# wxwilcke/mrgcn

Measured on AMD Instinct MI355X. Metric: full-batch R-GCN epoch time (ms), AM-shaped graph, lower is better.
Workload: dtype f32

## Files before the change

### mrgcn_amd/csrc/rgcn_fused.hip

```cpp
#include <cmath>
#include <cstdlib>

#include <mutex>
#include <unordered_map>

#include "common.hpp"
#include "config.hpp"

namespace mrgcn {
namespace {

constexpr int kTB = 256;
constexpr int kMixTB = 512;
constexpr int kMixFwdTB = 1024;
constexpr int kPre = 8;

__host__ __device__ constexpr int comp_stride(int BT) { return BT >= 4 ? BT + 4 : BT; }

template <int BT>
__device__ __forceinline__ void load_comp_row(const float *row, float (&w)[BT]) {
  if constexpr (BT % 4 == 0) {
#pragma unroll
    for (int b = 0; b < BT; b += 4) {
      const float4 q = *reinterpret_cast<const float4 *>(row + b);
      w[b] = q.x; w[b + 1] = q.y; w[b + 2] = q.z; w[b + 3] = q.w;
    }
  } else {
#pragma unroll
    for (int b = 0; b < BT; ++b) w[b] = row[b];
  }
}

template <int BT, typename OT>
__global__ __launch_bounds__(kMixFwdTB) void k_mix_fwd(const int32_t *__restrict__ nptr,
                                                    const int32_t *__restrict__ urel,
                                                    const int32_t *__restrict__ mpos,
                                                    const float *__restrict__ V,
                                                    const float *__restrict__ comp, int64_t N, int R,
                                                    int B, int b0, int F,
                                                    const float *__restrict__ addend, int64_t ldA,
                                                    OT *__restrict__ M, int64_t ldM, int accumulate,
                                                    int comp_in_lds,
                                                    const int32_t *__restrict__ node_ids = nullptr) {
  extern __shared__ __align__(16) float s_comp[];
  constexpr int CS = comp_stride(BT);
  const int nb = min(BT, B - b0);
  if (comp_in_lds) {
    for (int t = threadIdx.x; t < R * BT; t += blockDim.x) {
      int r = t / BT, b = t - r * BT;
      s_comp[r * CS + b] = (b < nb) ? comp[(int64_t)r * B + b0 + b] : 0.f;
    }
    __syncthreads();
  }
  const int64_t total = N * F;
  for (int64_t t = (int64_t)blockIdx.x * blockDim.x + threadIdx.x; t < total;
       t += (int64_t)gridDim.x * blockDim.x) {
    const int64_t j = t / F;
    const int o = (int)(t - j * F);
    const int32_t c0 = nptr[j], c1 = nptr[j + 1];
    if (c0 == c1) continue;
    float v[BT];
    const int64_t jv = node_ids ? (int64_t)node_ids[j] : j;
#pragma unroll
    for (int b = 0; b < BT; ++b)
      v[b] = (o < F && b < nb) ? V[(jv * B + (b0 + b)) * F + o] : 0.f;

    for (int32_t cb = c0; cb < c1; cb += kPre) {
      int rr[kPre];
      int32_t pp[kPre];
      float aa[kPre];
#pragma unroll
      for (int i = 0; i < kPre; ++i) {
        const int32_t c = (cb + i < c1) ? cb + i : cb;
        rr[i] = urel[c];
        pp[i] = mpos ? mpos[c] : c;
        aa[i] = addend ? addend[(int64_t)c * ldA + o] : 0.f;
      }
#pragma unroll
      for (int i = 0; i < kPre; ++i) {
        if (cb + i < c1) {
          float s = aa[i];
          if (comp_in_lds) {
            float w[BT];
            load_comp_row<BT>(s_comp + rr[i] * CS, w);
#pragma unroll
            for (int b = 0; b < BT; ++b) s = fmaf(w[b], v[b], s);
          } else {
            const float *cr = comp + (int64_t)rr[i] * B + b0;
#pragma unroll
            for (int b = 0; b < BT; ++b)
              if (b < nb) s = fmaf(cr[b], v[b], s);
          }
          OT *m = M + (int64_t)pp[i] * ldM + o;
          if (accumulate) s += load_operand<OT>(m);
          if constexpr (sizeof(OT) == 2) {
            const float next = __shfl_down(s, 1, kWave);
            if ((o & 1) == 0 && (F & 1) == 0) {
              *reinterpret_cast<uint32_t *>(m) = (uint32_t)f32_to_bf16(s) | ((uint32_t)f32_to_bf16(next) << 16);
            } else if (F & 1) {
              store_operand<OT>(m, s);
            }
          } else {
            store_operand<OT>(m, s);
          }
        }
      }
    }
  }
}

__device__ __forceinline__ void wave_lds_fence() {
  __builtin_amdgcn_fence(__ATOMIC_ACQ_REL, "wavefront");
  __builtin_amdgcn_wave_barrier();
}

using f32x4m = __attribute__((ext_vector_type(4))) float;
constexpr int kFwdTB = 1024;

template <int KS, bool NEAR, int ADD, typename OT, typename AT = float>
__device__ __forceinline__ void mix_node_tiles(int32_t c0, int32_t c1, int32_t base, int32_t ur, int32_t mp,
                                               const float (&pa)[4], const int32_t *__restrict__ urel,
                                               const int32_t *__restrict__ mpos, const float *s_comp,
                                               const float *s_v, int B, int F, const AT *__restrict__ addend,
                                               int64_t ldA, OT *__restrict__ M, int64_t ldM, int m, int kq,
                                               const AT *s_add = nullptr) {
  constexpr int KP = KS * 16 + 4;
  f32x4m bv[KS];
#pragma unroll
  for (int ks = 0; ks < KS; ++ks) {
    const int k0 = ks * 16 + 4 * kq;
    const float *t = s_v + k0 * F + m;
    bv[ks].x = (m < F && k0 + 0 < B) ? t[0] : 0.f;
    bv[ks].y = (m < F && k0 + 1 < B) ? t[F] : 0.f;
    bv[ks].z = (m < F && k0 + 2 < B) ? t[2 * F] : 0.f;
    bv[ks].w = (m < F && k0 + 3 < B) ? t[3 * F] : 0.f;
  }
  for (int32_t cb = c0; cb < c1; cb += 16) {
    const int32_t cm = cb + m;
    int32_t r;
    int32_t pos[4];
    f32x4m acc = f32x4m{0.f, 0.f, 0.f, 0.f};
    if (NEAR) {
      r = __shfl(ur, (cm - base) & 63);
#pragma unroll
      for (int reg = 0; reg < 4; ++reg) {
        pos[reg] = __shfl(mp, (cb - base + 4 * kq + reg) & 63);
        if (ADD == 1) acc[reg] = pa[reg];
        if (ADD == 2) acc[reg] = load_operand<AT>(s_add + (min(cb + 4 * kq + reg, c1 - 1) - base) * (int)ldA + min(m, F - 1));
      }
    } else {
      r = urel[min(cm, c1 - 1)];
#pragma unroll
      for (int reg = 0; reg < 4; ++reg) {
        const int32_t c = min(cb + 4 * kq + reg, c1 - 1);
        pos[reg] = mpos ? mpos[c] : c;
        if (ADD) acc[reg] = load_operand<AT>(addend + (int64_t)c * ldA + min(m, F - 1));
      }
    }
#pragma unroll
    for (int ks = 0; ks < KS; ++ks) {
      f32x4m av = *reinterpret_cast<const f32x4m *>(s_comp + r * KP + ks * 16 + 4 * kq);
      if (cm >= c1) av = f32x4m{0.f, 0.f, 0.f, 0.f};
      acc = __builtin_amdgcn_mfma_f32_16x16x4f32(av.x, bv[ks].x, acc, 0, 0, 0);
      acc = __builtin_amdgcn_mfma_f32_16x16x4f32(av.y, bv[ks].y, acc, 0, 0, 0);
      acc = __builtin_amdgcn_mfma_f32_16x16x4f32(av.z, bv[ks].z, acc, 0, 0, 0);
      acc = __builtin_amdgcn_mfma_f32_16x16x4f32(av.w, bv[ks].w, acc, 0, 0, 0);
    }
    if (m < F) {
#pragma unroll
      for (int reg = 0; reg < 4; ++reg)
        if (cb + 4 * kq + reg < c1) store_operand<OT>(M + (int64_t)pos[reg] * ldM + m, acc[reg]);
    }
    if (NEAR && ADD == 1) break;
  }
}

template <int BT>
__global__ __launch_bounds__(256) void k_mix_fwd_wide(const int32_t *__restrict__ nptr, const int32_t *__restrict__ urel,
                                                      const int32_t *__restrict__ mpos, const float *__restrict__ V,
                                                      const float *__restrict__ comp, int64_t N, int R, int B, int F,
                                                      float *__restrict__ M, int64_t ldM,
                                                      const int32_t *__restrict__ node_ids) {
  extern __shared__ __align__(16) float s_comp[];
  for (int t = threadIdx.x; t < R * B; t += blockDim.x) s_comp[t] = comp[t];
  __syncthreads();
  const int lane = threadIdx.x & 63;
  const int wv = __builtin_amdgcn_readfirstlane((int)(threadIdx.x >> 6));
  const int f0 = 4 * lane;
  const bool active = f0 < F;
  const f32x4m zero = {0.f, 0.f, 0.f, 0.f};
  for (int64_t j = (int64_t)blockIdx.x * 4 + wv; j < N; j += (int64_t)gridDim.x * 4) {
    const int32_t c0 = nptr[j], c1 = nptr[j + 1];
    if (c0 == c1) continue;
    const int64_t jv = node_ids ? (int64_t)node_ids[j] : j;
    f32x4m v[BT];
#pragma unroll
    for (int b = 0; b < BT; ++b)
      v[b] = (active && b < B) ? *reinterpret_cast<const f32x4m *>(V + (jv * B + b) * F + f0) : zero;
    for (int32_t cb = c0; cb < c1; cb += 64) {
      const int32_t my = (cb + lane < c1) ? cb + lane : c1 - 1;
      const int32_t mr = urel[my], mp = mpos ? mpos[my] : my;
      const int cnt = (c1 - cb < 64) ? c1 - cb : 64;
      for (int t = 0; t < cnt; ++t) {
        const int r = __builtin_amdgcn_readlane(mr, t);
        const int64_t pos = __builtin_amdgcn_readlane(mp, t);
        f32x4m sum = zero;
#pragma unroll
        for (int b = 0; b < BT; ++b)
          if (b < B) sum += v[b] * s_comp[r * B + b];
        if (active) *reinterpret_cast<f32x4m *>(M + pos * ldM + f0) = sum;
      }
    }
  }
}

#ifndef MIX_V_NT
#define MIX_V_NT 1
#endif
constexpr int kAddPieces = 128;
constexpr int kMixTile = 4;
template <int KS, int NQ, int TN, int ADD, typename OT, bool IDS = false, typename AT = float, bool TK = false>
__global__ __launch_bounds__(kFwdTB) void k_mix_fwd_mfma(
    const int32_t *__restrict__ nptr, const int32_t *__restrict__ urel, const int32_t *__restrict__ mpos,
    const float *__restrict__ V, const float *__restrict__ comp, int64_t N, int R, int B, int F,
    const AT *__restrict__ addend, int64_t ldA, OT *__restrict__ M, int64_t ldM,
    const int32_t *__restrict__ node_ids = nullptr, unsigned long long *__restrict__ tickets = nullptr,
    int n_counters = 0, int tile = kMixTile) {
  extern __shared__ __align__(16) float s_mem[];
  constexpr int KP = KS * 16 + 4;
  float *s_comp = s_mem;
  const int BF = B * F, nf4 = BF >> 2;
  const int lane = threadIdx.x & 63;
  const int wv = __builtin_amdgcn_readfirstlane((int)(threadIdx.x >> 6));
  const int nw = blockDim.x >> 6;
  float *s_tile = s_mem + ((R * KP + 3) & ~3) + wv * (TN * BF);
  float *s_add = s_mem + ((R * KP + 3) & ~3) + nw * (TN * BF) + wv * (kAddPieces * 4);
  const int q4 = (int)((ldA * (int64_t)sizeof(AT)) >> 4);
  for (int t = threadIdx.x; t < R * KP; t += blockDim.x) {
    const int r = t / KP, k = t - r * KP;
    s_comp[t] = k < B ? comp[(int64_t)r * B + k] : 0.f;
  }
  __syncthreads();
  const int m = lane & 15, kq = lane >> 4;
  const int64_t ngroups = (N + TN - 1) / TN;
  const int64_t nwaves = (int64_t)gridDim.x * nw;
  int64_t g = (int64_t)blockIdx.x * nw + wv, g1 = g + nwaves, g2 = g + 2 * nwaves;
  unsigned long long *ctr = nullptr;
  int64_t seg_lo = 0, seg_hi = 0;
  unsigned long long tk_ahead = 0;
  auto tile_first = [&](unsigned long long t) {
    const int64_t st = seg_lo + (int64_t)t * tile;
    return st < seg_hi ? st : ngroups;
  };
  auto next_step = [&](int64_t x) {
    if (x >= ngroups) return x;
    if ((x - seg_lo + 1) % tile != 0 && x + 1 < seg_hi) return x + 1;
    const unsigned long long t = __shfl(tk_ahead, 0, 64);
    if (lane == 0) tk_ahead = atomicAdd(ctr, 1ull);
    return tile_first(t);
  };
  if (TK) {
    const int64_t wid = g;
    const int c = (int)(wid % n_counters);
    ctr = tickets + (int64_t)c * kWorkTicketStride;
    const int64_t per = ((ngroups + n_counters - 1) / n_counters + tile - 1) / tile * tile;
    seg_lo = (int64_t)c * per;
    seg_hi = min(seg_lo + per, ngroups);
    unsigned long long t0 = 0;
    if (lane == 0) {
      t0 = atomicAdd(ctr, 1ull);
      tk_ahead = atomicAdd(ctr, 1ull);
    }
    g = tile_first(__shfl(t0, 0, 64));
    g1 = next_step(g);
    g2 = next_step(g1);
  }
  if (g >= ngroups) return;
#define MIX_LOAD_NP(gg) nptr[min(min((gg), ngroups - 1) * TN + min(lane, TN), N)]
#define MIX_LOAD_ID(gg) (IDS ? node_ids[min(min((gg), ngroups - 1) * TN + min(lane, TN - 1), N - 1)] : 0)
#define MIX_LOAD_V(gg, idreg)                                                                               \
  _Pragma("unroll") for (int i = 0; i < TN; ++i) {                                                          \
    const int64_t nid = IDS ? (int64_t)__builtin_amdgcn_readlane(idreg, i) : min((gg) * TN + i, N - 1);     \
    const f32x4m *src = reinterpret_cast<const f32x4m *>(V) + nid * (int64_t)nf4;                           \
    _Pragma("unroll") for (int q = 0; q < NQ; ++q)                                                          \
      pv[i][q] = MIX_V_NT ? __builtin_nontemporal_load(src + min(lane + 64 * q, nf4 - 1)) : src[min(lane + 64 * q, nf4 - 1)]; \
  }
#define MIX_LOAD_IDX(np, ur, mp)                                                                            \
  {                                                                                                         \
    const int32_t a0 = __builtin_amdgcn_readlane(np, 0), a1 = __builtin_amdgcn_readlane(np, TN);            \
    const int32_t ci = max(min(a0 + lane, a1 - 1), 0);                                                      \
    ur = urel[ci];                                                                                          \
    mp = mpos ? mpos[ci] : ci;                                                                              \
    if (ADD == 2) {                                                                                         \
      const int64_t p0 = (int64_t)a0 * q4, p1 = (int64_t)a1 * q4;                                           \
      const f32x4m *a4 = reinterpret_cast<const f32x4m *>(addend);                                          \
      pa4_n1[0] = a4[max(min(p0 + lane, p1 - 1), (int64_t)0)];                                              \
      pa4_n1[1] = a4[max(min(p0 + 64 + lane, p1 - 1), (int64_t)0)];                                         \
    }                                                                                                       \
    if (ADD == 1) {                                                                                         \
      _Pragma("unroll") for (int i = 0; i < TN; ++i) {                                                      \
        const int32_t b0 = __builtin_amdgcn_readlane(np, i), b1 = __builtin_amdgcn_readlane(np, i + 1);     \
        _Pragma("unroll") for (int reg = 0; reg < 4; ++reg) pa_n1[i][reg] =                                 \
            load_operand<AT>(addend + (int64_t)max(min(b0 + 4 * kq + reg, b1 - 1), 0) * ldA + min(m, F - 1)); \
      }                                                                                                     \
    }                                                                                                       \
  }
  f32x4m pv[TN][NQ];
  f32x4m pa4_n1[2];
  float pa_n1[TN][4], pa_cur[TN][4];
  int32_t np_cur = MIX_LOAD_NP(g), np_n1 = MIX_LOAD_NP(g1);
  int32_t id_cur = MIX_LOAD_ID(g), id_n1 = MIX_LOAD_ID(g1);
  int32_t ur_cur, mp_cur, ur_n1, mp_n1;
  MIX_LOAD_IDX(np_cur, ur_n1, mp_n1)
  MIX_LOAD_V(g, id_cur)
  for (; g < ngroups; g = g1, g1 = g2, g2 = TK ? next_step(g2) : g2 + nwaves) {
    const int32_t np_now = np_cur;
    const int32_t cbase = __builtin_amdgcn_readlane(np_now, 0), cend = __builtin_amdgcn_readlane(np_now, TN);
    const int32_t np_n2 = MIX_LOAD_NP(g2);
    const int32_t id_n2 = MIX_LOAD_ID(g2);
    ur_cur = ur_n1;
    mp_cur = mp_n1;
    bool near = cend - cbase <= 64;
    if (ADD == 2) near = near && (cend - cbase) * q4 <= kAddPieces;
#pragma unroll
    for (int i = 0; i < TN; ++i) {
      if (ADD == 1) {
#pragma unroll
        for (int reg = 0; reg < 4; ++reg) pa_cur[i][reg] = pa_n1[i][reg];
        near = near && __builtin_amdgcn_readlane(np_now, i + 1) - __builtin_amdgcn_readlane(np_now, i) <= 16;
      }
      f32x4m *dst = reinterpret_cast<f32x4m *>(s_tile + i * BF);
#pragma unroll
      for (int q = 0; q < NQ; ++q)
        if (lane + 64 * q < nf4) dst[lane + 64 * q] = pv[i][q];
    }
    if (ADD == 2) {
      reinterpret_cast<f32x4m *>(s_add)[lane] = pa4_n1[0];
      reinterpret_cast<f32x4m *>(s_add)[64 + lane] = pa4_n1[1];
    }
    wave_lds_fence();
    MIX_LOAD_V(g1, id_n1)
    MIX_LOAD_IDX(np_n1, ur_n1, mp_n1)
    np_cur = np_n1;
    np_n1 = np_n2;
    id_n1 = id_n2;
    if (near) {
#pragma unroll
      for (int i = 0; i < TN; ++i) {
        const int32_t c0 = __builtin_amdgcn_readlane(np_now, i), c1 = __builtin_amdgcn_readlane(np_now, i + 1);
        if (c1 > c0)
          mix_node_tiles<KS, true, ADD, OT, AT>(c0, c1, cbase, ur_cur, mp_cur, pa_cur[i], urel, mpos, s_comp,
                                                s_tile + i * BF, B, F, addend, ldA, M, ldM, m, kq,
                                                reinterpret_cast<const AT *>(s_add));
      }
    } else {
#pragma unroll 1
      for (int i = 0; i < TN; ++i)
        mix_node_tiles<KS, false, ADD, OT, AT>(__builtin_amdgcn_readlane(np_now, i),
                                               __builtin_amdgcn_readlane(np_now, i + 1), cbase, ur_cur, mp_cur,
                                               pa_cur[0], urel, mpos, s_comp, s_tile + i * BF, B, F, addend, ldA, M,
                                               ldM, m, kq);
    }
    wave_lds_fence();
  }
#undef MIX_LOAD_NP
#undef MIX_LOAD_ID
#undef MIX_LOAD_V
#undef MIX_LOAD_IDX
}

template <int BT>
__global__ __launch_bounds__(kMixTB) void k_mix_bwd_dv(const int32_t *__restrict__ nptr,
                                                       const int32_t *__restrict__ urel,
                                                       const float *__restrict__ dM, int64_t ldM,
                                                       const float *__restrict__ comp, int64_t N, int R,
                                                       int B, int b0, int F, float *__restrict__ dV,
                                                       int comp_in_lds, double *__restrict__ sumsq) {
  extern __shared__ __align__(16) float s_comp[];
  float sq = 0.f;
  constexpr int CS = comp_stride(BT);
  const int nb = min(BT, B - b0);
  if (comp_in_lds) {
    for (int t = threadIdx.x; t < R * BT; t += blockDim.x) {
      int r = t / BT, b = t - r * BT;
      s_comp[r * CS + b] = (b < nb) ? comp[(int64_t)r * B + b0 + b] : 0.f;
    }
    __syncthreads();
  }
  const int64_t total = N * F;
  for (int64_t t = (int64_t)blockIdx.x * blockDim.x + threadIdx.x; t < total;
       t += (int64_t)gridDim.x * blockDim.x) {
    const int64_t j = t / F;
    const int o = (int)(t - j * F);
    const int32_t c0 = nptr[j], c1 = nptr[j + 1];
    float acc[BT];
#pragma unroll
    for (int b = 0; b < BT; ++b) acc[b] = 0.f;
    for (int32_t cb = c0; cb < c1; cb += kPre) {
      int rr[kPre];
      float dd[kPre];
#pragma unroll
      for (int i = 0; i < kPre; ++i) {
        const bool in = cb + i < c1;
        rr[i] = in ? urel[cb + i] : 0;
        dd[i] = in ? dM[(int64_t)(cb + i) * ldM + o] : 0.f;
      }
#pragma unroll
      for (int i = 0; i < kPre; ++i) {
        if (cb + i < c1) {
          if (comp_in_lds) {
            float w[BT];
            load_comp_row<BT>(s_comp + rr[i] * CS, w);
#pragma unroll
            for (int b = 0; b < BT; ++b) acc[b] = fmaf(w[b], dd[i], acc[b]);
          } else {
            const float *cr = comp + (int64_t)rr[i] * B + b0;
#pragma unroll
            for (int b = 0; b < BT; ++b)
              if (b < nb) acc[b] = fmaf(cr[b], dd[i], acc[b]);
          }
        }
      }
    }
#pragma unroll
    for (int b = 0; b < BT; ++b)
      if (b < nb) {
        dV[((int64_t)j * B + (b0 + b)) * F + o] = acc[b];
        sq = fmaf(acc[b], acc[b], sq);
      }
  }
  if (sumsq) {
    __shared__ float s_sq[kMixTB / 64];
#pragma unroll
    for (int off = 32; off > 0; off >>= 1) sq += __shfl_xor(sq, off, 64);
    if ((threadIdx.x & 63) == 0) s_sq[threadIdx.x >> 6] = sq;
    __syncthreads();
    if (threadIdx.x == 0) {
      float t = 0.f;
      for (int i = 0; i < (int)(blockDim.x >> 6); ++i) t += s_sq[i];
      atomicAdd(sumsq, (double)t);
    }
  }
}

constexpr int kNodeTB = 1024;
constexpr int kNodeLaunchTB = 512;
static_assert(kNodeLaunchTB % 64 == 0 && kNodeLaunchTB <= kNodeTB && 4 * kNodeLaunchTB <= 2048, "whole waves; four blocks per CU");
constexpr int kGroup = 4;

typedef float f32x4_a8 __attribute__((ext_vector_type(4), aligned(8)));
template <int FT>
__device__ __forceinline__ void load_row(const float *__restrict__ p, int F, float (&v)[FT]) {
  if ((F & 1) == 0) {
#pragma unroll
    for (int o = 0; o < FT; o += 4) {
      if (o + 4 <= F && o + 4 <= FT) {
        const f32x4_a8 t = *reinterpret_cast<const f32x4_a8 *>(p + o);
        v[o] = t.x;
        v[o + 1] = t.y;
        v[o + 2] = t.z;
        v[o + 3] = t.w;
      } else {
#pragma unroll
        for (int u = o; u < o + 4 && u < FT; u += 2) {
          if (u < F) {
            const float2 t = *reinterpret_cast<const float2 *>(p + u);
            v[u] = t.x;
            if (u + 1 < FT) v[u + 1] = t.y;
          } else {
            v[u] = 0.f;
            if (u + 1 < FT) v[u + 1] = 0.f;
          }
        }
      }
    }
  } else {
#pragma unroll
    for (int o = 0; o < FT; ++o) v[o] = (o < F) ? p[o] : 0.f;
  }
}
template <int FT>
__device__ __forceinline__ void store_row_f(float *__restrict__ p, int F, const float (&v)[FT]) {
  if ((F & 1) == 0) {
#pragma unroll
    for (int o = 0; o < FT; o += 2)
      if (o < F) *reinterpret_cast<float2 *>(p + o) = make_float2(v[o], (o + 1 < FT) ? v[o + 1] : 0.f);
  } else {
#pragma unroll
    for (int o = 0; o < FT; ++o)
      if (o < F) p[o] = v[o];
  }
}

template <int FT>
__global__ __launch_bounds__(kNodeTB) void k_mix_bwd_nm(const int32_t *__restrict__ nptr,
                                                        const int32_t *__restrict__ urel,
                                                        const float *__restrict__ dM, int64_t ldM,
                                                        const float *__restrict__ V,
                                                        const float *__restrict__ comp, int64_t N, int R,
                                                        int B, int F, float *__restrict__ dV,
                                                        float *__restrict__ dcomp,
                                                        double *__restrict__ sumsq, int top_rel,
                                                        const uint8_t *__restrict__ col_live,
                                                        uint8_t *__restrict__ node_cur, int dc_in_lds) {
  extern __shared__ __align__(16) float s_dc[];
  const int lane = threadIdx.x & 63;
  const int wv = __builtin_amdgcn_readfirstlane((int)(threadIdx.x >> 6));
  const int nw = blockDim.x >> 6;
  if (dc_in_lds) {
    for (int t = threadIdx.x; t < R * B; t += blockDim.x) s_dc[t] = 0.f;
    __syncthreads();
  }
  const bool on = lane < B;
  const int b = on ? lane : 0;
// ... 686 lines not shown
                                                      const int32_t *__restrict__ unode,
                                                      const float *__restrict__ X, int64_t ldX, int K,
                                                      const float *__restrict__ dM, int64_t ldM, int F,
                                                      float *__restrict__ dW) {
  extern __shared__ float smem[];
  const int chunk = blockIdx.x;
  const int r = relchunk_rel[chunk];
  const int32_t beg = relchunk_beg[chunk], end = relchunk_end[chunk];
  __shared__ int32_t s_c[kTK], s_j[kTK];
  const int XS = kKS + 1;
  float *Xs = smem;
  float *Ds = smem + kTK * XS;
  float *dWr = dW + (int64_t)r * K * F;

  for (int k0 = 0; k0 < K; k0 += kKS) {
    const int ks = min(kKS, K - k0);
    const int npairs = ks * F;
    for (int pbase = 0; pbase < npairs; pbase += kTB * kPP) {
      float acc[kPP];
#pragma unroll
      for (int q = 0; q < kPP; ++q) acc[q] = 0.f;
      for (int32_t t0 = beg; t0 < end; t0 += kTK) {
        const int nk = min(kTK, end - t0);
        __syncthreads();
        if (threadIdx.x < nk) {
          int32_t c = rperm[t0 + threadIdx.x];
          s_c[threadIdx.x] = c;
          s_j[threadIdx.x] = unode[c];
        }
        __syncthreads();
        for (int t = threadIdx.x; t < nk * ks; t += kTB) {
          int kk = t / ks, i = t - kk * ks;
          Xs[kk * XS + i] = X[(int64_t)s_j[kk] * ldX + k0 + i];
        }
        for (int t = threadIdx.x; t < nk * F; t += kTB) {
          int kk = t / F, o = t - kk * F;
          Ds[t] = dM[(int64_t)s_c[kk] * ldM + o];
        }
        __syncthreads();
#pragma unroll
        for (int q = 0; q < kPP; ++q) {
          const int p = pbase + q * kTB + threadIdx.x;
          if (p < npairs) {
            const int i = p / F, o = p - i * F;
            float s = acc[q];
            for (int kk = 0; kk < nk; ++kk) s = fmaf(Xs[kk * XS + i], Ds[kk * F + o], s);
            acc[q] = s;
          }
        }
      }
#pragma unroll
      for (int q = 0; q < kPP; ++q) {
        const int p = pbase + q * kTB + threadIdx.x;
        if (p < npairs) atomicAdd(&dWr[(int64_t)k0 * F + p], acc[q]);
      }
    }
  }
}

__global__ __launch_bounds__(kTB) void k_xform_bwd_dx(const int32_t *__restrict__ nptr,
                                                      const int32_t *__restrict__ urel,
                                                      const float *__restrict__ dM, int64_t ldM,
                                                      const float *__restrict__ W, int64_t N, int K,
                                                      int F, float *__restrict__ dX, int64_t lddX) {
  const int64_t total = N * K;
  for (int64_t t = (int64_t)blockIdx.x * blockDim.x + threadIdx.x; t < total;
       t += (int64_t)gridDim.x * blockDim.x) {
    const int64_t j = t / K;
    const int i = (int)(t - j * K);
    const int32_t c0 = nptr[j], c1 = nptr[j + 1];
    float s = 0.f;
    for (int32_t c = c0; c < c1; ++c) {
      const float *w = W + ((int64_t)urel[c] * K + i) * F;
      const float *dm = dM + (int64_t)c * ldM;
      for (int o = 0; o < F; ++o) s = fmaf(dm[o], w[o], s);
    }
    dX[j * lddX + i] = s;
  }
}

int grid_for(int64_t work_items, int tb = kTB, int max_blocks = 256 * 8) {
  int64_t b = (work_items + tb - 1) / tb;
  if (b < 1) b = 1;
  if (b > max_blocks) b = max_blocks;
  return (int)b;
}

constexpr size_t kLdsBudget = 64 * 1024;

bool use_mfma() {
  const bool v = cfg(CFG_XFORM_MFMA) != 0;
  return v;
}

int mix_grid(size_t lds, int64_t work_items) {
  int per_cu = lds > 0 ? (int)((160 * 1024) / (lds + 256)) : 4;
  if (per_cu > 4) per_cu = 4;
  if (per_cu < 1) per_cu = 1;
  int64_t want = (work_items + kMixTB - 1) / kMixTB;
  int64_t grid = 256 * per_cu * 2;
  if (grid > want) grid = want;
  return (int)(grid < 1 ? 1 : grid);
}

}
}

using namespace mrgcn;

namespace {

struct MixCols {
  const int32_t *nptr, *urel, *mpos, *node_ids;
  int64_t N, ncols;
  int R;
  unsigned long long *tickets = nullptr;
};

template <typename OT, typename AT = float>
int mix_fwd_cols(const MixCols *p, const float *V, const float *comp, int32_t B, int32_t F,
                 const AT *addend, int64_t ldA, OT *M, int64_t ldM, void *stream) {
  MRGCN_REQUIRE(V && comp && M, "NULL");
  MRGCN_REQUIRE(B > 0 && F > 0 && ldM >= F, "B / F / ldM");
  MRGCN_REQUIRE(!addend || ldA >= F, "ldA");
  if (p->ncols == 0 || p->N == 0) return MRGCN_OK;
  hipStream_t s = (hipStream_t)stream;
  const int R = p->R;
  const int64_t N = p->N;
  const int32_t *node_ids = p->node_ids;
  const int32_t *mpos_arg = p->mpos;
  if constexpr (sizeof(OT) == 4) {
    const bool wide_on = cfg(CFG_MIX_WIDE) != 0;
    if (wide_on && !addend && F > 16 && F <= 256 && F % 4 == 0 && B <= 4 && ldM % 4 == 0 &&
        ((((uintptr_t)V) | ((uintptr_t)M)) & 15) == 0 && (size_t)R * B * sizeof(float) <= 64 * 1024) {
      const size_t lds = (size_t)R * B * sizeof(float);
      int64_t grid = (N + 3) / 4;
      if (grid > 256 * 8) grid = 256 * 8;
#define MIXW_GO(BT_)                                                                                            \
  k_mix_fwd_wide<BT_><<<dim3((unsigned)grid), dim3(256), lds, s>>>(p->nptr, p->urel, mpos_arg, V, comp, N, R, B, F, \
                                                                    (float *)M, ldM, node_ids)
      if (B == 1) MIXW_GO(1);
      else if (B == 2) MIXW_GO(2);
      else MIXW_GO(4);
#undef MIXW_GO
      MRGCN_HIP_TRY(hipGetLastError());
      return MRGCN_OK;
    }
  }
  {
    const bool mfma_on = cfg(CFG_MIX_MFMA) != 0;
    constexpr int tn = 2;
    const int KS = (B + 15) / 16;
    const int NQ = (B * F + 255) / 256;
    const size_t lds_plain =
        ((size_t)((R * (KS * 16 + 4) + 3) & ~3) + (size_t)(kFwdTB / 64) * tn * B * F) * sizeof(float);
    const size_t lds_add = (size_t)(kFwdTB / 64) * kAddPieces * 4 * sizeof(float);
    const bool add_vec = addend && (ldA * sizeof(AT)) % 16 == 0 && ldA <= 16 && (((uintptr_t)addend) & 15) == 0 &&
                         !node_ids && cfg(CFG_MIX_ADD_VEC) != 0 &&
                         lds_plain + lds_add <= 150 * 1024;
    const size_t lds = lds_plain + (add_vec ? lds_add : 0);
    if (mfma_on && B <= 64 && F <= 16 && (B * F) % 4 == 0 && (((uintptr_t)V) & 15) == 0 &&
        lds <= 150 * 1024 && !(node_ids && (addend || sizeof(OT) != 4))) {
      const int64_t want = ((N + tn - 1) / tn + (kFwdTB / 64) - 1) / (kFwdTB / 64);
      int64_t grid = 256;
      if (grid > want) grid = want;
      const int n_ctr = (int)std::min<int64_t>(std::max<int64_t>(cfg(CFG_MIX_TICKETS), 0), kWorkTickets);
      const int tk_tile = (int)std::min<int64_t>(std::max<int64_t>(cfg(CFG_MIX_TICKET_TILE), 1), 64);
      const int64_t mix_steps = (N + tn - 1) / tn;
      const bool tk = p->tickets && !node_ids && n_ctr > 0 && grid == 256 &&
                      mix_steps >= (int64_t)4 * tk_tile * grid * (kFwdTB / 64);
      if (tk)
        MRGCN_HIP_TRY(mrgcn::fill_async(p->tickets, 0, (size_t)kWorkTickets * kWorkTicketStride * sizeof(unsigned long long), s));
#define MIXM_GO(KS_, NQ_, TN_)                                                                              \
  do {                                                                                                      \
    auto kfn = addend ? (add_vec ? k_mix_fwd_mfma<KS_, NQ_, TN_, 2, OT, false, AT>                          \
                                 : k_mix_fwd_mfma<KS_, NQ_, TN_, 1, OT, false, AT>)                         \
                      : k_mix_fwd_mfma<KS_, NQ_, TN_, 0, OT, false, AT>;                                    \
    if (tk) kfn = addend ? (add_vec ? k_mix_fwd_mfma<KS_, NQ_, TN_, 2, OT, false, AT, true>                 \
                                    : k_mix_fwd_mfma<KS_, NQ_, TN_, 1, OT, false, AT, true>)                \
                         : k_mix_fwd_mfma<KS_, NQ_, TN_, 0, OT, false, AT, true>;                           \
    if constexpr (sizeof(OT) == 4 && sizeof(AT) == 4) if (node_ids) kfn = k_mix_fwd_mfma<KS_, NQ_, TN_, 0, OT, true>; \
    MRGCN_HIP_TRY(raise_lds_limit((const void *)kfn, lds));  \
    kfn<<<dim3((unsigned)grid), dim3(kFwdTB), lds, s>>>(p->nptr, p->urel, mpos_arg, V, comp, N, R, B, F,     \
                                                        addend, ldA, M, ldM, node_ids, p->tickets,          \
                                                        n_ctr, tk_tile);                                    \
  } while (0)
#define MIXM_TN(KS_, NQ_) MIXM_GO(KS_, NQ_, tn)
      switch (KS * 8 + NQ) {
        case 1 * 8 + 1: MIXM_TN(1, 1); break;
        case 2 * 8 + 1: MIXM_TN(2, 1); break;
        case 2 * 8 + 2: MIXM_TN(2, 2); break;
        case 3 * 8 + 1: MIXM_TN(3, 1); break;
        case 3 * 8 + 2: MIXM_TN(3, 2); break;
        case 3 * 8 + 3: MIXM_TN(3, 3); break;
        case 4 * 8 + 1: MIXM_TN(4, 1); break;
        case 4 * 8 + 2: MIXM_TN(4, 2); break;
        case 4 * 8 + 3: MIXM_TN(4, 3); break;
        default: MIXM_TN(4, 4); break;
      }
#undef MIXM_TN
#undef MIXM_GO
      MRGCN_HIP_TRY(hipGetLastError());
      return MRGCN_OK;
    }
  }
  if constexpr (sizeof(AT) != 4) {
    set_error("basis mix with a bf16 addend: outside the matrix-core form's limits (B <= 64, F <= 16, B*F % 4 == 0)");
    return MRGCN_ERR_UNSUPPORTED;
  } else {
  int acc = 0;
  for (int b0 = 0; b0 < B; b0 += 64) {
    const int nb = (B - b0 < 64) ? (B - b0) : 64;
    int BT = nb <= 2 ? 2 : nb <= 4 ? 4 : nb <= 8 ? 8 : nb <= 16 ? 16 : nb <= 32 ? 32 : nb <= 40 ? 40 : 64;
    size_t lds = (size_t)R * comp_stride(BT) * sizeof(float);
    int in_lds = lds <= kLdsBudget;
    if (!in_lds) lds = 0;
    int grid = mix_grid(lds, N * F);
    const float *add = acc ? nullptr : addend;
#define MIX_GO(T)                                                                                    \
  k_mix_fwd<T, OT><<<dim3(grid), dim3(kMixFwdTB), lds, s>>>(p->nptr, p->urel, mpos_arg, V, comp, N, R, B, b0, \
                                                        F, add, ldA, M, ldM, acc, in_lds, node_ids)
    switch (BT) {
      case 2: MIX_GO(2); break;
      case 4: MIX_GO(4); break;
      case 8: MIX_GO(8); break;
      case 16: MIX_GO(16); break;
      case 32: MIX_GO(32); break;
      case 40: MIX_GO(40); break;
      default: MIX_GO(64); break;
    }
#undef MIX_GO
    MRGCN_HIP_TRY(hipGetLastError());
    acc = 1;
  }
  return MRGCN_OK;
  }
}

template <typename OT>
int mix_fwd_impl(const mrgcn_plan_t *p, const float *V, const float *comp, int32_t B, int32_t F,
                 const float *addend, int64_t ldA, OT *M, int64_t ldM, void *stream) {
  MRGCN_REQUIRE(p, "NULL");
  const MixCols c{p->nptr, p->urel, p->mpos, nullptr, p->num_nodes, p->ncols, (int)p->num_relations,
                  p->work_tickets};
  return mix_fwd_cols<OT>(&c, V, comp, B, F, addend, ldA, M, ldM, stream);
}
}

namespace mrgcn {
int mix_fwd_arrays(const int32_t *nptr, const int32_t *urel, const int32_t *node_ids, int64_t n_nodes, int64_t ncols,
                   int R, const float *V, const float *comp, int32_t B, int32_t F, float *M, int64_t ldM,
                   hipStream_t s) {
  const MixCols c{nptr, urel, nullptr, node_ids, n_nodes, ncols, R};
  return mix_fwd_cols<float, float>(&c, V, comp, B, F, (const float *)nullptr, 0, M, ldM, (void *)s);
}
}

namespace {

__global__ __launch_bounds__(kTB) void k_basis_contract(const float *__restrict__ comp, const float *__restrict__ V,
                                                        int R, int B, int64_t X, float *__restrict__ W) {
  const int64_t total = (int64_t)R * X;
  for (int64_t t = (int64_t)blockIdx.x * kTB + threadIdx.x; t < total; t += (int64_t)gridDim.x * kTB) {
    const int64_t r = t / X, x = t - r * X;
    const float *c = comp + r * B;
    float s0 = 0.f, s1 = 0.f;
    int b = 0;
    for (; b + 2 <= B; b += 2) {
      s0 = fmaf(c[b], V[(int64_t)b * X + x], s0);
      s1 = fmaf(c[b + 1], V[(int64_t)(b + 1) * X + x], s1);
    }
    if (b < B) s0 = fmaf(c[b], V[(int64_t)b * X + x], s0);
    W[t] = s0 + s1;
  }
}

constexpr int kContractMaxB = 64;
template <int BT, int NW = 4>
__global__ __launch_bounds__(64 * NW) void k_basis_contract_bwd(const float *__restrict__ comp, const float *__restrict__ V,
                                                            const float *__restrict__ dW, int R, int B, int64_t X,
                                                            float *__restrict__ dcomp, float *__restrict__ dV,
                                                            int dv_blocks, int tiled) {
  constexpr int kTB = 64 * NW;
  extern __shared__ float s_mem[];
  {
    if (!tiled) {
      const int64_t total = (int64_t)B * X;
      for (int64_t t = (int64_t)blockIdx.x * kTB + threadIdx.x; t < total; t += (int64_t)dv_blocks * kTB) {
        const int64_t b = t / X, x = t - b * X;
        float s0 = 0.f, s1 = 0.f;
        int r = 0;
        for (; r + 2 <= R; r += 2) {
          s0 = fmaf(comp[(int64_t)r * B + b], dW[(int64_t)r * X + x], s0);
          s1 = fmaf(comp[(int64_t)(r + 1) * B + b], dW[(int64_t)(r + 1) * X + x], s1);
        }
        if (r < R) s0 = fmaf(comp[(int64_t)r * B + b], dW[(int64_t)r * X + x], s0);
        dV[t] = s0 + s1;
      }
      return;
    }
    float *s_comp = s_mem;
    float *s_part = s_mem + (size_t)R * BT;
    for (int t0 = 0; t0 < R * BT; t0 += kTB * 8) {
      float v[8];
#pragma unroll
      for (int u = 0; u < 8; ++u) {
        const int t = t0 + u * kTB + threadIdx.x;
        const int r = t / BT, b = t - r * BT;
        v[u] = (t < R * BT && b < B) ? comp[(int64_t)r * B + b] : 0.f;
      }
#pragma unroll
      for (int u = 0; u < 8; ++u) {
        const int t = t0 + u * kTB + threadIdx.x;
// ... 610 lines not shown
```

Measured before the change: 4.755.

## Transpose MFMA mix output to row-major lanes with vectorized stores and register addend

Swaps the MFMA operand order so each lane holds four consecutive feature columns of one output row, which allows vectorized row-group stores and loads in place of four scalar strided stores per lane. The ADD==2 addend is now kept in registers and fetched by cross-lane shuffles instead of being staged through a per-wave LDS region. That region is removed from the LDS budget, which may raise occupancy. Ticket broadcasts use readfirstlane instead of shfl. The cost is extra shuffle and select logic, plus unaligned vector stores at odd widths.

```diff
diff --git a/mrgcn_amd/csrc/rgcn_fused.hip b/mrgcn_amd/csrc/rgcn_fused.hip
--- a/mrgcn_amd/csrc/rgcn_fused.hip
+++ b/mrgcn_amd/csrc/rgcn_fused.hip
@@ -114,16 +114,87 @@
   __builtin_amdgcn_wave_barrier();
 }
 
+__device__ __forceinline__ unsigned long long wave_first(unsigned long long x) {
+  const uint32_t lo = (uint32_t)__builtin_amdgcn_readfirstlane((int)(uint32_t)x);
+  const uint32_t hi = (uint32_t)__builtin_amdgcn_readfirstlane((int)(uint32_t)(x >> 32));
+  return ((unsigned long long)hi << 32) | lo;
+}
+
 using f32x4m = __attribute__((ext_vector_type(4))) float;
 constexpr int kFwdTB = 1024;
 
+typedef f32x4m f32x4u __attribute__((aligned(4)));
+typedef __attribute__((ext_vector_type(3))) float f32x3m;
+typedef f32x3m f32x3u __attribute__((aligned(4)));
+typedef __attribute__((ext_vector_type(2))) float f32x2m;
+typedef f32x2m f32x2u __attribute__((aligned(4)));
+typedef __attribute__((ext_vector_type(2))) uint32_t u32x2m;
+typedef u32x2m u32x2u __attribute__((aligned(4)));
+typedef __attribute__((ext_vector_type(4))) uint16_t u16x4m;
+typedef u16x4m u16x4u __attribute__((aligned(2)));
+
+#ifndef MIX_M_NT
+#define MIX_M_NT 0
+#endif
+template <typename OT>
+__device__ __forceinline__ void store_row_group(OT *p, const f32x4m &v, int n, bool even) {
+  if constexpr (sizeof(OT) == 4) {
+#if MIX_M_NT
+#define MIX_ST(T, val) __builtin_nontemporal_store(val, reinterpret_cast<T *>(p))
+#else
+#define MIX_ST(T, val) *reinterpret_cast<T *>(p) = val
+#endif
+    if (n == 4) MIX_ST(f32x4u, v);
+    else if (n == 3) MIX_ST(f32x3u, (f32x3m{v.x, v.y, v.z}));
+    else if (n == 2) MIX_ST(f32x2u, (f32x2m{v.x, v.y}));
+    else MIX_ST(float, v.x);
+#undef MIX_ST
+  } else {
+    const uint32_t h0 = f32_to_bf16(v.x), h1 = f32_to_bf16(v.y), h2 = f32_to_bf16(v.z), h3 = f32_to_bf16(v.w);
+    if (even) {
+      const uint32_t w0 = h0 | (h1 << 16), w1 = h2 | (h3 << 16);
+      if (n == 4) *reinterpret_cast<u32x2u *>(p) = u32x2m{w0, w1};
+      else if (n >= 2) *reinterpret_cast<uint32_t *>(p) = w0;
+      if (n == 3) p[2] = (uint16_t)h2;
+      if (n == 1) p[0] = (uint16_t)h0;
+    } else {
+      p[0] = (uint16_t)h0;
+      if (n > 1) p[1] = (uint16_t)h1;
+      if (n > 2) p[2] = (uint16_t)h2;
+      if (n > 3) p[3] = (uint16_t)h3;
+    }
+  }
+}
+
+template <typename AT>
+__device__ __forceinline__ f32x4m load_row_group(const AT *row, int q, int F, int ld) {
+  float e[4];
+  if (ld >= 4) {
+    const int fs = max(min(4 * q, ld - 4), 0), sh = 4 * q - fs;
+    if constexpr (sizeof(AT) == 4) {
+      const f32x4m v = *reinterpret_cast<const f32x4u *>(row + fs);
+      e[0] = v.x; e[1] = v.y; e[2] = v.z; e[3] = v.w;
+    } else {
+      const u16x4m v = *reinterpret_cast<const u16x4u *>(row + fs);
+      e[0] = bf16_to_f32(v.x); e[1] = bf16_to_f32(v.y); e[2] = bf16_to_f32(v.z); e[3] = bf16_to_f32(v.w);
+    }
+    e[0] = sh == 0 ? e[0] : sh == 1 ? e[1] : sh == 2 ? e[2] : e[3];
+    e[1] = sh == 0 ? e[1] : sh == 1 ? e[2] : e[3];
+    e[2] = sh == 0 ? e[2] : e[3];
+  } else {
+#pragma unroll
+    for (int i = 0; i < 4; ++i) e[i] = load_operand<AT>(row + min(4 * q + i, F - 1));
+  }
+  return f32x4m{e[0], e[1], e[2], e[3]};
+}
+
 template <int KS, bool NEAR, int ADD, typename OT, typename AT = float>
 __device__ __forceinline__ void mix_node_tiles(int32_t c0, int32_t c1, int32_t base, int32_t ur, int32_t mp,
-                                               const float (&pa)[4], const int32_t *__restrict__ urel,
+                                               const f32x4m &pa, const f32x4m (&pa4)[2], int q4,
+                                               const int32_t *__restrict__ urel,
                                                const int32_t *__restrict__ mpos, const float *s_comp,
                                                const float *s_v, int B, int F, const AT *__restrict__ addend,
-                                               int64_t ldA, OT *__restrict__ M, int64_t ldM, int m, int kq,
-                                               const AT *s_add = nullptr) {
+                                               int64_t ldA, OT *__restrict__ M, int64_t ldM, int m, int kq) {
   constexpr int KP = KS * 16 + 4;
   f32x4m bv[KS];
 #pragma unroll
@@ -135,42 +206,47 @@
     bv[ks].z = (m < F && k0 + 2 < B) ? t[2 * F] : 0.f;
     bv[ks].w = (m < F && k0 + 3 < B) ? t[3 * F] : 0.f;
   }
+  const int nf = min(F - 4 * kq, 4);
+  const bool even = (ldM & 1) == 0 && (reinterpret_cast<uintptr_t>(M) & 3) == 0;
   for (int32_t cb = c0; cb < c1; cb += 16) {
     const int32_t cm = cb + m;
-    int32_t r;
-    int32_t pos[4];
+    const int32_t cc = min(cm, c1 - 1);
+    int32_t r, pos;
     f32x4m acc = f32x4m{0.f, 0.f, 0.f, 0.f};
     if (NEAR) {
-      r = __shfl(ur, (cm - base) & 63);
-#pragma unroll
-      for (int reg = 0; reg < 4; ++reg) {
-        pos[reg] = __shfl(mp, (cb - base + 4 * kq + reg) & 63);
-        if (ADD == 1) acc[reg] = pa[reg];
-        if (ADD == 2) acc[reg] = load_operand<AT>(s_add + (min(cb + 4 * kq + reg, c1 - 1) - base) * (int)ldA + min(m, F - 1));
+      r = __shfl(ur, (cc - base) & 63);
+      pos = __shfl(mp, (cc - base) & 63);
+      if (ADD == 1) acc = pa;
+      if (ADD == 2) {
+        const int pi = (cc - base) * q4 + min(sizeof(AT) == 4 ? kq : kq >> 1, q4 - 1);
+        float w[4];
+#pragma unroll
+        for (int i = 0; i < 4; ++i) {
+          const float lo = __shfl(pa4[0][i], pi & 63), hi = __shfl(pa4[1][i], pi & 63);
+          w[i] = pi < 64 ? lo : hi;
+        }
+        if constexpr (sizeof(AT) == 4) {
+          acc = f32x4m{w[0], w[1], w[2], w[3]};
+        } else {
+          const uint32_t u0 = __float_as_uint((kq & 1) ? w[2] : w[0]), u1 = __float_as_uint((kq & 1) ? w[3] : w[1]);
+          acc = f32x4m{__uint_as_float(u0 << 16), __uint_as_float(u0 & 0xffff0000u), __uint_as_float(u1 << 16),
+                       __uint_as_float(u1 & 0xffff0000u)};
+        }
       }
     } else {
-      r = urel[min(cm, c1 - 1)];
-#pragma unroll
-      for (int reg = 0; reg < 4; ++reg) {
-        const int32_t c = min(cb + 4 * kq + reg, c1 - 1);
-        pos[reg] = mpos ? mpos[c] : c;
-        if (ADD) acc[reg] = load_operand<AT>(addend + (int64_t)c * ldA + min(m, F - 1));
-      }
+      r = urel[cc];
+      pos = mpos ? mpos[cc] : cc;
+      if (ADD) acc = load_row_group<AT>(addend + (int64_t)cc * ldA, kq, F, (int)ldA);
     }
 #pragma unroll
     for (int ks = 0; ks < KS; ++ks) {
-      f32x4m av = *reinterpret_cast<const f32x4m *>(s_comp + r * KP + ks * 16 + 4 * kq);
-      if (cm >= c1) av = f32x4m{0.f, 0.f, 0.f, 0.f};
-      acc = __builtin_amdgcn_mfma_f32_16x16x4f32(av.x, bv[ks].x, acc, 0, 0, 0);
-      acc = __builtin_amdgcn_mfma_f32_16x16x4f32(av.y, bv[ks].y, acc, 0, 0, 0);
-      acc = __builtin_amdgcn_mfma_f32_16x16x4f32(av.z, bv[ks].z, acc, 0, 0, 0);
-      acc = __builtin_amdgcn_mfma_f32_16x16x4f32(av.w, bv[ks].w, acc, 0, 0, 0);
-    }
-    if (m < F) {
-#pragma unroll
-      for (int reg = 0; reg < 4; ++reg)
-        if (cb + 4 * kq + reg < c1) store_operand<OT>(M + (int64_t)pos[reg] * ldM + m, acc[reg]);
-    }
+      const f32x4m av = *reinterpret_cast<const f32x4m *>(s_comp + r * KP + ks * 16 + 4 * kq);
+      acc = __builtin_amdgcn_mfma_f32_16x16x4f32(bv[ks].x, av.x, acc, 0, 0, 0);
+      acc = __builtin_amdgcn_mfma_f32_16x16x4f32(bv[ks].y, av.y, acc, 0, 0, 0);
+      acc = __builtin_amdgcn_mfma_f32_16x16x4f32(bv[ks].z, av.z, acc, 0, 0, 0);
+      acc = __builtin_amdgcn_mfma_f32_16x16x4f32(bv[ks].w, av.w, acc, 0, 0, 0);
+    }
+    if (cm < c1 && nf > 0) store_row_group<OT>(M + (int64_t)pos * ldM + 4 * kq, acc, nf, even);
     if (NEAR && ADD == 1) break;
   }
 }
@@ -234,7 +310,6 @@
   const int wv = __builtin_amdgcn_readfirstlane((int)(threadIdx.x >> 6));
   const int nw = blockDim.x >> 6;
   float *s_tile = s_mem + ((R * KP + 3) & ~3) + wv * (TN * BF);
-  float *s_add = s_mem + ((R * KP + 3) & ~3) + nw * (TN * BF) + wv * (kAddPieces * 4);
   const int q4 = (int)((ldA * (int64_t)sizeof(AT)) >> 4);
   for (int t = threadIdx.x; t < R * KP; t += blockDim.x) {
     const int r = t / KP, k = t - r * KP;
@@ -255,7 +330,7 @@
   auto next_step = [&](int64_t x) {
     if (x >= ngroups) return x;
     if ((x - seg_lo + 1) % tile != 0 && x + 1 < seg_hi) return x + 1;
-    const unsigned long long t = __shfl(tk_ahead, 0, 64);
+    const unsigned long long t = wave_first(tk_ahead);
     if (lane == 0) tk_ahead = atomicAdd(ctr, 1ull);
     return tile_first(t);
   };
@@ -271,7 +346,7 @@
       t0 = atomicAdd(ctr, 1ull);
       tk_ahead = atomicAdd(ctr, 1ull);
     }
-    g = tile_first(__shfl(t0, 0, 64));
+    g = tile_first(wave_first(t0));
     g1 = next_step(g);
     g2 = next_step(g1);
   }
@@ -300,14 +375,13 @@
     if (ADD == 1) {                                                                                         \
       _Pragma("unroll") for (int i = 0; i < TN; ++i) {                                                      \
         const int32_t b0 = __builtin_amdgcn_readlane(np, i), b1 = __builtin_amdgcn_readlane(np, i + 1);     \
-        _Pragma("unroll") for (int reg = 0; reg < 4; ++reg) pa_n1[i][reg] =                                 \
-            load_operand<AT>(addend + (int64_t)max(min(b0 + 4 * kq + reg, b1 - 1), 0) * ldA + min(m, F - 1)); \
+        pa_n1[i] = load_row_group<AT>(addend + (int64_t)max(min(b0 + m, b1 - 1), 0) * ldA, kq, F, (int)ldA);  \
       }                                                                                                     \
     }                                                                                                       \
   }
   f32x4m pv[TN][NQ];
-  f32x4m pa4_n1[2];
-  float pa_n1[TN][4], pa_cur[TN][4];
+  f32x4m pa4_n1[2], pa4_cur[2];
+  f32x4m pa_n1[TN], pa_cur[TN];
   int32_t np_cur = MIX_LOAD_NP(g), np_n1 = MIX_LOAD_NP(g1);
   int32_t id_cur = MIX_LOAD_ID(g), id_n1 = MIX_LOAD_ID(g1);
   int32_t ur_cur, mp_cur, ur_n1, mp_n1;
@@ -325,8 +399,7 @@
 #pragma unroll
     for (int i = 0; i < TN; ++i) {
       if (ADD == 1) {
-#pragma unroll
-        for (int reg = 0; reg < 4; ++reg) pa_cur[i][reg] = pa_n1[i][reg];
+        pa_cur[i] = pa_n1[i];
         near = near && __builtin_amdgcn_readlane(np_now, i + 1) - __builtin_amdgcn_readlane(np_now, i) <= 16;
       }
       f32x4m *dst = reinterpret_cast<f32x4m *>(s_tile + i * BF);
@@ -335,8 +408,9 @@
         if (lane + 64 * q < nf4) dst[lane + 64 * q] = pv[i][q];
     }
     if (ADD == 2) {
-      reinterpret_cast<f32x4m *>(s_add)[lane] = pa4_n1[0];
-      reinterpret_cast<f32x4m *>(s_add)[64 + lane] = pa4_n1[1];
+      pa4_cur[0] = pa4_n1[0];
+      pa4_cur[1] = pa4_n1[1];
+      asm volatile("" : "+v"(pa4_cur[0]), "+v"(pa4_cur[1]));
     }
     wave_lds_fence();
     MIX_LOAD_V(g1, id_n1)
@@ -349,17 +423,16 @@
       for (int i = 0; i < TN; ++i) {
         const int32_t c0 = __builtin_amdgcn_readlane(np_now, i), c1 = __builtin_amdgcn_readlane(np_now, i + 1);
         if (c1 > c0)
-          mix_node_tiles<KS, true, ADD, OT, AT>(c0, c1, cbase, ur_cur, mp_cur, pa_cur[i], urel, mpos, s_comp,
-                                                s_tile + i * BF, B, F, addend, ldA, M, ldM, m, kq,
-                                                reinterpret_cast<const AT *>(s_add));
+          mix_node_tiles<KS, true, ADD, OT, AT>(c0, c1, cbase, ur_cur, mp_cur, pa_cur[i], pa4_cur, q4, urel, mpos,
+                                                s_comp, s_tile + i * BF, B, F, addend, ldA, M, ldM, m, kq);
       }
     } else {
 #pragma unroll 1
       for (int i = 0; i < TN; ++i)
         mix_node_tiles<KS, false, ADD, OT, AT>(__builtin_amdgcn_readlane(np_now, i),
                                                __builtin_amdgcn_readlane(np_now, i + 1), cbase, ur_cur, mp_cur,
-                                               pa_cur[0], urel, mpos, s_comp, s_tile + i * BF, B, F, addend, ldA, M,
-                                               ldM, m, kq);
+                                               pa_cur[0], pa4_cur, q4, urel, mpos, s_comp, s_tile + i * BF, B, F,
+                                               addend, ldA, M, ldM, m, kq);
     }
     wave_lds_fence();
   }
@@ -1352,13 +1425,10 @@
     constexpr int tn = 2;
     const int KS = (B + 15) / 16;
     const int NQ = (B * F + 255) / 256;
-    const size_t lds_plain =
+    const size_t lds =
         ((size_t)((R * (KS * 16 + 4) + 3) & ~3) + (size_t)(kFwdTB / 64) * tn * B * F) * sizeof(float);
-    const size_t lds_add = (size_t)(kFwdTB / 64) * kAddPieces * 4 * sizeof(float);
     const bool add_vec = addend && (ldA * sizeof(AT)) % 16 == 0 && ldA <= 16 && (((uintptr_t)addend) & 15) == 0 &&
-                         !node_ids && cfg(CFG_MIX_ADD_VEC) != 0 &&
-                         lds_plain + lds_add <= 150 * 1024;
-    const size_t lds = lds_plain + (add_vec ? lds_add : 0);
+                         !node_ids && cfg(CFG_MIX_ADD_VEC) != 0;
     if (mfma_on && B <= 64 && F <= 16 && (B * F) % 4 == 0 && (((uintptr_t)V) & 15) == 0 &&
         lds <= 150 * 1024 && !(node_ids && (addend || sizeof(OT) != 4))) {
       const int64_t want = ((N + tn - 1) / tn + (kFwdTB / 64) - 1) / (kFwdTB / 64);
```

Result: no change. 4.773 (+0.4%).
